# podmortem/log-parser

Hardware: AMD Instinct MI355X
Metric: log-lines/sec parsed+scored (whole node), 1k-pattern library (higher is better)
Workload: dtype fp64

## Files before the change

### csrc/bind.cpp

```cpp
#include <pybind11/numpy.h>
#include <pybind11/pybind11.h>
#include <pybind11/stl.h>

#include <atomic>
#include <chrono>
#include <condition_variable>
#include <cstring>
#include <deque>
#include <memory>
#include <mutex>
#include <thread>

#include "io/docs.h"
#include "io/json_in.h"
#include "io/loadgen.h"
#include "io/http_server.h"
#include "io/json_emit.h"
#include "kernels/lp_api.h"
#include "kernels/lp_host.h"
#include "regex/jregex.h"
#include "runtime/proc_shared.h"
#include "runtime/request.h"

namespace py = pybind11;
// ... 884 lines not shown
    bool intact = true;
    for (size_t i = k; i < out.size(); ++i) intact = intact && out[i] == '\xAB';
    return py::make_tuple(py::bytes(out.data(), k), intact);
  });

  m.def("line_index_tiles", &line_index_tiles);
  m.def("line_index_dev", [](uint64_t text, int64_t n, uint64_t ws, int64_t ntiles_cap, uint64_t starts, uint64_t lens,
                             int64_t cap, uint64_t info, bool trim, uint64_t blk, int64_t nblk, uint64_t s, bool counted) {
    line_index_dev(P<const uint8_t>(text), n, LineIndexWs{P<int64_t>(ws), ntiles_cap, size_t(1) << 20}, P<int64_t>(starts),
                   P<int32_t>(lens), cap, P<int64_t>(info), trim, P<int32_t>(blk), nblk, s, counted); },
        py::arg("text"), py::arg("n"), py::arg("ws"), py::arg("ntiles_cap"), py::arg("starts"), py::arg("lens"),
        py::arg("cap"), py::arg("info"), py::arg("trim"), py::arg("blk"), py::arg("nblk"), py::arg("s"),
        py::arg("counted") = false);
  m.def("prefilter_dev", [](uint64_t text, int64_t n, py::tuple pf, uint64_t ls, int64_t nl, uint64_t cand, int64_t cap,
                            uint64_t count, int grid, uint64_t s, py::object nlp) {
    NlOut o;
    const bool fused = !nlp.is_none();
    if (fused) {
      py::tuple t = nlp.cast<py::tuple>();
      o.nlm = P<uint64_t>(t[0].cast<uint64_t>());
      o.cnt = P<int32_t>(t[1].cast<uint64_t>());
      o.crf = P<int32_t>(t[2].cast<uint64_t>());
      o.ntiles = t[3].cast<int64_t>();
    }
    prefilter_dev(P<const uint8_t>(text), n, pf_from(pf), P<const int64_t>(ls), nl, P<int64_t>(cand), cap,
                  P<unsigned long long>(count), grid, s, fused ? &o : nullptr); },
        py::arg("text"), py::arg("n"), py::arg("pf"), py::arg("ls"), py::arg("nl"), py::arg("cand"), py::arg("cap"),
        py::arg("count"), py::arg("grid"), py::arg("s"), py::arg("nlp") = py::none());
  m.def("line_index_pass1", [](uint64_t ws, int64_t ntiles_cap, int64_t n, uint64_t s) {
    const NlOut o = line_index_pass1_views(LineIndexWs{P<int64_t>(ws), ntiles_cap, size_t(1) << 20}, n, s);
    return py::make_tuple(reinterpret_cast<uint64_t>(o.nlm), reinterpret_cast<uint64_t>(o.cnt),
                          reinterpret_cast<uint64_t>(o.crf), o.ntiles);
  });
  m.def("pf_verify_dev", [](uint64_t gh, int64_t n, uint64_t text, int64_t nb, py::tuple pf, uint64_t ls, int64_t nl,
                            uint64_t blk, uint64_t cand, int64_t cap, uint64_t count, uint64_t s, uint64_t dn,
                            int max_grid) {
    pf_verify_dev(P<const int64_t>(gh), n, P<const uint8_t>(text), nb, pf_from(pf), P<const int64_t>(ls), nl,
                  P<const int32_t>(blk), P<int64_t>(cand), cap, P<unsigned long long>(count), s,
                  P<const unsigned long long>(dn), max_grid); }, py::arg("gh"), py::arg("n"), py::arg("text"),
        py::arg("nb"), py::arg("pf"), py::arg("ls"), py::arg("nl"), py::arg("blk"), py::arg("cand"), py::arg("cap"),
        py::arg("count"), py::arg("s"), py::arg("dn") = 0, py::arg("max_grid") = 8192);
  m.def("append_keys", [](uint64_t dst, int64_t cap, uint64_t count, uint64_t src, int64_t n, uint64_t s) {
    append_keys_dev(P<int64_t>(dst), cap, P<unsigned long long>(count), P<const int64_t>(src), n, s); });
  m.def("take_host", [](uint64_t cand, uint64_t n1d, int64_t cap1, uint64_t ver, uint64_t n2d, int64_t cap2,
                        uint64_t text, uint64_t ls, uint64_t ll, py::tuple dfa, py::object out, uint64_t s) {
    HostSideOut O;
    if (!out.is_none()) {
      py::tuple t = out.cast<py::tuple>();
      O.keys = P<int64_t>(t[0].cast<uint64_t>()); O.starts = P<int64_t>(t[1].cast<uint64_t>());
      O.lens = P<int64_t>(t[2].cast<uint64_t>()); O.cap = t[3].cast<int64_t>();
      O.cnt = P<unsigned long long>(t[4].cast<uint64_t>()); O.done_blocks = P<unsigned int>(t[5].cast<uint64_t>());
      O.host_cnt = P<int64_t>(t[6].cast<uint64_t>()); O.host_seq = P<int64_t>(t[7].cast<uint64_t>());
      O.seq = t[8].cast<int64_t>();
    }
    take_host_dev(P<int64_t>(cand), P<const unsigned long long>(n1d), cap1, P<int64_t>(ver),
                  P<const unsigned long long>(n2d), cap2, P<const uint8_t>(text), P<const int64_t>(ls),
                  P<const int32_t>(ll), dfa_from(dfa), O, s); });
  m.def("wait_host", [](uint64_t ver, int64_t cap2, uint64_t n2d, py::tuple in, uint64_t s, double timeout_s) {
    HostSideIn I;
    I.keys = P<const int64_t>(in[0].cast<uint64_t>()); I.host_cnt = P<const int64_t>(in[1].cast<uint64_t>());
    I.host_seq = P<const int64_t>(in[2].cast<uint64_t>()); I.cap = in[3].cast<int64_t>(); I.seq = in[4].cast<int64_t>();
    I.err = P<int64_t>(in[5].cast<uint64_t>());
    I.timeout_ticks = (long long)(timeout_s * 1e8);
    wait_host_dev(P<int64_t>(ver), cap2, P<unsigned long long>(n2d), I, s); }, py::arg("ver"), py::arg("cap2"),
    py::arg("n2d"), py::arg("in"), py::arg("stream"), py::arg("timeout_s") = 2.0);
  m.def("host_alloc_coherent", [](int64_t bytes) {
// ... 284 lines not shown
        py::arg("hist"), py::arg("stream"), py::arg("dev"));
  m.def("trace_tile", &trace_tile);
  m.def("trace_runs_tmp_bytes", &trace_runs_tmp_bytes, py::arg("L"));
  m.def("trace_class", [](uint64_t text, int64_t tbytes, uint64_t ls, uint64_t ll, int64_t L, uint64_t cls, uint64_t elem,
                          uint64_t s, bool dev) {
    if (dev) {
      trace_class_dev(P<const uint8_t>(text), tbytes, P<const int64_t>(ls), P<const int32_t>(ll), L, P<uint8_t>(cls),
                      P<uint64_t>(elem), s);
      return;
    }
    py::gil_scoped_release nogil;
    trace_class_host(P<const uint8_t>(text), tbytes, P<const int64_t>(ls), P<const int32_t>(ll), L, P<uint8_t>(cls),
                     P<uint64_t>(elem)); },
        py::arg("text"), py::arg("tbytes"), py::arg("ls"), py::arg("ll"), py::arg("L"), py::arg("cls"), py::arg("elem"),
        py::arg("stream"), py::arg("dev"));
  m.def("trace_runs", [](uint64_t cls, uint64_t elem, uint64_t evm, int64_t L, std::vector<int64_t> carry, bool last,
                         uint64_t out, int64_t cap, uint64_t cnt, uint64_t carry_out, uint64_t tmp, uint64_t s, bool dev) {
    if ((int)carry.size() != TR_CARRY_WORDS) throw std::runtime_error("trace_runs: the carry has 13 words");
    TraceRunArgs A;
    A.cls = P<const uint8_t>(cls); A.elem = P<const uint64_t>(elem); A.evm = P<const uint8_t>(evm); A.L = L;
    A.in = TrCarry{carry[0], (uint64_t)carry[1], (uint64_t)carry[2], carry[3], carry[4], carry[5], carry[6], carry[7],
                   carry[8], carry[9], carry[10], carry[11], carry[12]};
    A.last = last;
    A.out = P<int64_t>(out); A.cap = cap; A.cnt = P<unsigned long long>(cnt); A.carry_out = P<int64_t>(carry_out);
    if (dev) {
      trace_runs_dev(A, P<void>(tmp), s);
      return;
    }
    py::gil_scoped_release nogil;
    trace_runs_host(A); },
        py::arg("cls"), py::arg("elem"), py::arg("evm"), py::arg("L"), py::arg("carry"), py::arg("last"), py::arg("out"),
        py::arg("cap"), py::arg("cnt"), py::arg("carry_out"), py::arg("tmp"), py::arg("stream"), py::arg("dev"));
  m.def("scan_multi", [](uint64_t text, int64_t nbytes, uint64_t ls, uint64_t ll, int64_t nl, py::tuple pass,
                         uint64_t out, int64_t cap, uint64_t cnt, int grid, uint64_t s, bool dev) -> int64_t {
    const ScanPass S = scan_pass_from(pass);
    if (dev) {
      scan_multi_dev(P<const uint8_t>(text), nbytes, P<const int64_t>(ls), P<const int32_t>(ll), nl, S, P<int64_t>(out), cap,
                     P<unsigned long long>(cnt), grid, s);
      return 0;
    }
    py::gil_scoped_release nogil;
    return scan_multi_host(P<const uint8_t>(text), P<const int64_t>(ls), P<const int32_t>(ll), nl, S, P<int64_t>(out),
                           cap);
  });
  m.def("freq_evict", [](py::tuple ring, double horizon, uint64_t s, bool dev) {
    freq_evict(ring_from(ring), horizon, s, dev);
  });
  m.def("summarize", [](py::tuple in, int64_t n, int k, int nsev, uint64_t top, uint64_t pat_hist, uint64_t sev_hist,
                        uint64_t ws, uint64_t ws_bytes, uint64_t s, bool dev) -> uint64_t {
    const SummIn I{P<const double>(in[0].cast<uint64_t>()), P<const int32_t>(in[1].cast<uint64_t>()),
                   P<const int32_t>(in[2].cast<uint64_t>()), P<const int64_t>(in[3].cast<uint64_t>()),
                   P<const int64_t>(in[4].cast<uint64_t>()), P<const int32_t>(in[5].cast<uint64_t>()),
                   P<const double>(in[6].cast<uint64_t>()),
                   in.size() > 7 ? P<void>(in[7].cast<uint64_t>()) : nullptr,
                   in.size() > 8 ? P<const int64_t>(in[8].cast<uint64_t>()) : nullptr};
    if (dev)
      return summarize_dev(I, n, k, nsev, P<double>(top), P<unsigned long long>(pat_hist), P<unsigned long long>(sev_hist),
                           P<void>(ws), ws_bytes, s);
    summarize_host(I, n, k, P<double>(top), P<int64_t>(pat_hist), P<int64_t>(sev_hist));
    return 0;
  });
  m.def("rescore", [](uint64_t gl, uint64_t fac, int64_t n, int64_t Nn, py::tuple sp, uint64_t out, uint64_t s,
                      bool dev) {
    if (dev)
      rescore_dev(P<const int64_t>(gl), P<const double>(fac), n, Nn, sp_from(sp), P<double>(out), s);
    else
      rescore_host(P<const int64_t>(gl), P<const double>(fac), n, Nn, sp_from(sp), P<double>(out));
  });
  m.def("dp_pack", [](int64_t own_lines, uint64_t freq, int nk, uint64_t chain, int ns, uint64_t pack, uint64_t s,
                      bool dev, uint64_t cnt, std::vector<int64_t> caps) {
    if (cnt && caps.size() != 4) throw std::invalid_argument("dp_pack: 4 capacities");
    dp_pack(own_lines, P<const int64_t>(freq), nk, P<const int32_t>(chain), ns, P<int64_t>(pack), s, dev,
            P<const int64_t>(cnt), cnt ? caps.data() : nullptr); },
        py::arg("own_lines"), py::arg("freq"), py::arg("nk"), py::arg("chain"), py::arg("ns"), py::arg("pack"),
        py::arg("s"), py::arg("dev"), py::arg("cnt") = 0, py::arg("caps") = std::vector<int64_t>());
  m.def("dp_carry", [](py::tuple a, uint64_t s, bool dev) {
    auto u = [&](int i) { return a[i].cast<uint64_t>(); };
// ... 454 lines not shown
```

### csrc/kernels/line_index.hip

```cpp
#include <hip/hip_runtime.h>

#include <cstring>
#include <stdexcept>
#include <string>

#include "lp_api.h"

namespace lp {

constexpr int LI_BYTES_PER_THREAD = 64;
__device__ __forceinline__ uint32_t li_zero_bytes(uint32_t t) {
  const uint32_t y = (t & 0x7F7F7F7Fu) + 0x7F7F7F7Fu;
  return ~(y | t | 0x7F7F7F7Fu);
}

constexpr int LI_THREADS = 256;
constexpr int LI_TILE = LI_THREADS * LI_BYTES_PER_THREAD;
constexpr int LI_STAGE = LI_THREADS * 8;

__device__ __forceinline__ int li_masks(const uint8_t* __restrict__ text, int64_t nbytes, int64_t base,
                                        uint32_t (&m)[16], uint32_t (&cr)[16]) {
  int c = 0;
  if (base < nbytes) {
    const uint4* p = reinterpret_cast<const uint4*>(text + base);
// ... 293 lines not shown
    for (int k = 0; k < LS_PER; ++k) {
      o[k] = run;
      run += cur[k];
    }
    if (i0 + LS_PER <= nt && ((uintptr_t)off & 15) == 0) {
      longlong2* o2 = reinterpret_cast<longlong2*>(off + i0);
#pragma unroll
      for (int k = 0; k < LS_PER / 2; ++k) o2[k] = make_longlong2(o[2 * k], o[2 * k + 1]);
    } else {
#pragma unroll
      for (int k = 0; k < LS_PER; ++k)
        if (i0 + k < nt) off[i0 + k] = o[k];
    }
    carry += tot;
#pragma unroll
    for (int k = 0; k < LS_PER; ++k) cur[k] = nxt[k];
  }
}

int64_t line_index_tiles(int64_t nbytes) { return (nbytes + LI_TILE - 1) / LI_TILE; }

NlOut line_index_pass1_views(const LineIndexWs& W, int64_t nbytes, uint64_t stream) {
  const int64_t nt = line_index_tiles(nbytes);
  if (nt <= 0 || nt > W.ntiles_cap) throw std::runtime_error("line_index: empty text or workspace too small");
  NlOut o;
  o.cnt = reinterpret_cast<int32_t*>(W.buf + 3 * W.ntiles_cap);
  o.crf = o.cnt + W.ntiles_cap;
  o.nlm = reinterpret_cast<uint64_t*>(W.buf + 4 * W.ntiles_cap);
  o.ntiles = nt;
  const hipError_t e = hipMemsetAsync(o.cnt, 0, (size_t)(W.ntiles_cap + nt) * sizeof(int32_t),
                                      reinterpret_cast<hipStream_t>(stream));
  if (e != hipSuccess) throw std::runtime_error(std::string("HIP error: ") + hipGetErrorString(e) + " in line_index");
  return o;
}

void line_index_dev(const uint8_t* text, int64_t nbytes, const LineIndexWs& W, int64_t* starts, int32_t* lens,
                    int64_t cap, int64_t* info, bool trim, int32_t* blk, int64_t nblk, uint64_t stream, bool counted) {
  const int64_t nt = line_index_tiles(nbytes);
  if (nt <= 0 || nt > W.ntiles_cap) throw std::runtime_error("line_index: empty text or workspace too small");
  hipStream_t st = reinterpret_cast<hipStream_t>(stream);
  int64_t* off = W.buf;
  int64_t* fix_g = W.buf + W.ntiles_cap;
  int64_t* fix_end = W.buf + 2 * W.ntiles_cap;
  int32_t* cnt = reinterpret_cast<int32_t*>(W.buf + 3 * W.ntiles_cap);
  int32_t* crf = cnt + W.ntiles_cap;
  uint64_t* nlm = reinterpret_cast<uint64_t*>(W.buf + 4 * W.ntiles_cap);
  if (!counted) hipLaunchKernelGGL(k_nl_count, dim3((unsigned)nt), dim3(LI_THREADS), 0, st, text, nbytes, cnt, nlm, crf);
  hipLaunchKernelGGL(k_tile_scan, dim3(1), dim3(LS_THREADS), 0, st, cnt, nt, off);
  hipLaunchKernelGGL(k_nl_lines, dim3((unsigned)((nt + LI_LINES_TPB - 1) / LI_LINES_TPB)), dim3(LI_THREADS), 0, st,
                     text, nbytes, (int64_t)nt, nlm, crf, off, starts, lens, cap,
                     fix_g, fix_end, blk, nblk);
  hipLaunchKernelGGL(k_line_fix, dim3((unsigned)((nt + 1 + 255) / 256)), dim3(256), 0, st, nt, nbytes, fix_g, fix_end,
                     off, cnt, starts, lens, cap, info, blk, nblk);
  if (trim) hipLaunchKernelGGL(k_line_trim, dim3(1), dim3(256), 0, st, lens, cap, info);
  const hipError_t e = hipGetLastError();
  if (e != hipSuccess) throw std::runtime_error(std::string("HIP error: ") + hipGetErrorString(e) + " in line_index");
}

}
```

### csrc/kernels/lp_api.h

```cpp
#pragma once
#include <stdint.h>

#include <vector>

#include "lp_core.h"

namespace lp {

void set_host_threads(int n);
void set_pf_verify_lanes(int n);
bool scan_defer_rare();
void set_scan_defer_rare(bool on);
void set_cand_verify_split(bool on);
bool summ_select();
void set_summ_select(bool on);
void set_small_profile(uint64_t dev_ptr);
struct NlOut {
  uint64_t* nlm = nullptr;
  int32_t* cnt = nullptr;
  int32_t* crf = nullptr;
  int64_t ntiles = 0;
};
void prefilter_dev(const uint8_t* text, int64_t nbytes, const PfTables& T, const int64_t* line_start, int64_t nlines,
                   int64_t* cand, int64_t cap, unsigned long long* count, int grid, uint64_t stream,
// ... 66 lines not shown
                const ScoreTables& T, const ScoreParams& S, double* out, double* factors);

}

namespace lp {
void nfa_mfma_dev(const uint64_t* groups, const int32_t* group_list, int ngroups, int ncls, const int32_t* lines,
                  int64_t nsel, const uint8_t* text, const int64_t* line_start, const int32_t* line_len,
                  uint8_t* feat, int64_t* hits, int64_t cap, unsigned long long* count, uint64_t stream);
int64_t nfa_host(const uint64_t* groups, const int32_t* group_list, int ngroups, const int32_t* lines, int64_t nsel,
                 const uint8_t* text, const int64_t* line_start, const int32_t* line_len, uint8_t* feat,
                 int64_t* hits, int64_t cap);
}

namespace lp {
struct ScanPass {
  const uint32_t* blob;
  int lds_words;
  int ngroups;
  int row_base[4];
  int stride[4];
  int thr[4];
  int init_row[4];
  uint32_t init_state[4];
  int ncol[4];
  int gt_off[4];
  int gm_off[4];
  int fin_off[4];
  int bm_off;
  int rid_off;
  int am_off;
};
void scan_multi_dev(const uint8_t* text, int64_t nbytes, const int64_t* line_start, const int32_t* line_len, int64_t nlines,
                    const ScanPass& S, int64_t* out, int64_t cap, unsigned long long* count, int grid,
                    uint64_t stream);
int64_t scan_multi_host(const uint8_t* text, const int64_t* line_start, const int32_t* line_len, int64_t nlines,
                        const ScanPass& S, int64_t* out, int64_t cap);
}

namespace lp {
struct FreqRing {
  double* t;
  int32_t* key;
  int32_t* cnt;
  int64_t cap;
  int64_t* ht;
  int64_t* tot;
  uint8_t* seen;
};
void freq_evict(const FreqRing& R, double horizon, uint64_t stream, bool dev);
struct RecordGate {
  const int64_t* cnt = nullptr;
  int64_t cap[4] = {0, 0, 0, 0};
  const int64_t* veto = nullptr;
};
void freq_record(const int64_t* counts, int K, double now, const FreqRing& R, uint64_t stream, bool dev,
                 const RecordGate& gate = RecordGate());
}

namespace lp {
struct LineIndexWs {
  int64_t* buf;
  int64_t ntiles_cap;
  size_t tmp_bytes;
};
int64_t line_index_tiles(int64_t nbytes);
void line_index_dev(const uint8_t* text, int64_t nbytes, const LineIndexWs& W, int64_t* starts, int32_t* lens,
                    int64_t cap, int64_t* info, bool trim, int32_t* blk, int64_t nblk, uint64_t stream,
                    bool counted = false);
NlOut line_index_pass1_views(const LineIndexWs& W, int64_t nbytes, uint64_t stream);
}

namespace lp {
struct DpCarryArgs {
  const int64_t* g;
  int world, rank, nk, ns;
  int64_t halo_left;
  const int64_t* tot;
  const int64_t* slot_e0;
  const int64_t* slot_k;
  int64_t* own_start; int64_t* g0; int64_t* n;
  int64_t* carry;
  uint8_t* seq_carry;
  int64_t* red_tail;
  int64_t* veto = nullptr;
  int64_t* zero = nullptr;
  int64_t nzero = 0;
  const uint8_t* seq_base = nullptr;
  int64_t line_base = 0;
  int64_t n_fixed = 0;
  uint8_t* seq_next = nullptr;
};
void dp_pack(int64_t own_lines, const int64_t* freq, int nk, const int32_t* chain, int ns, int64_t* pack,
             uint64_t stream, bool dev, const int64_t* cnt = nullptr, const int64_t* caps = nullptr);
void dp_carry(const DpCarryArgs& A, uint64_t stream, bool dev);
}

namespace lp {
struct SummIn {
  const double* score;
  const int32_t* pat;
  const int32_t* line32;
  const int64_t* line64;
// ... 279 lines not shown
```

### csrc/kernels/scan_multi.hip

```cpp
#include <hip/hip_runtime.h>

#include <map>
#include <mutex>
#include <stdexcept>
#include <string>
#include <utility>
#include <vector>

#include "lp_api.h"
#include "lp_core.h"
#include "lp_host.h"

namespace lp {

constexpr int SCAN_THREADS = 1024;
constexpr int SCAN_THREADS_SMALL = 256;
constexpr int SCAN_RUN = 4;
constexpr int SCAN_BM_COPIES = 32;
constexpr int SCAN_BM_REP_BYTES = 256 * SCAN_BM_COPIES * 4;

typedef __attribute__((address_space(3))) const uint16_t lds_u16_t;
typedef __attribute__((address_space(3))) const uint32_t lds_u32_t;
__device__ __forceinline__ uint32_t lds_ld16(uint32_t a) { return *(lds_u16_t*)(uintptr_t)a; }
__device__ __forceinline__ uint32_t lds_ld32(uint32_t a) { return *(lds_u32_t*)(uintptr_t)a; }
// ... 192 lines not shown
      } else {
        b = lds_ld32(c * 4);
      }
#pragma unroll
      for (int g = 0; g < G; ++g) {
        mx[g] = max(mx[g], xr[g]);
        xr[g] = lds_ld16(xr[g] + ((b >> (8 * g)) & 0xFFu));
      }
    }
    uint32_t hotm = 0;
#pragma unroll
    for (int g = 0; g < G; ++g) hotm |= (mx[g] >= (uint32_t)S.thr[g] ? 1u : 0u) << g;
    while (hotm) {
      const int g = __builtin_ctz(hotm);
      hotm &= hotm - 1;
      uint32_t xg = xs[0];
#pragma unroll
      for (int q = 1; q < G; ++q)
        if (g == q) xg = xs[q];
      if constexpr (DEFER) rare_push(rare, p0, p_lo, p_end, x0, x1, g, CRLF, xg);
      else scan_block_masks<CRLF>(S, w, hold, p0, p_lo, p_end, x0, x1, line_start, g, xg, emit);
    }
    cur = nxt;
    nxt = nx2;
  }
}

template <int G, int THREADS, bool DEFER>
__global__ __launch_bounds__(THREADS) void k_scan_multi(const uint8_t* __restrict__ text, int64_t nbytes,
                                                        const int64_t* __restrict__ line_start,
                                                        const int32_t* __restrict__ line_len, int64_t nlines,
                                                        ScanPass S, int64_t* __restrict__ out, int64_t cap,
                                                        unsigned long long* __restrict__ count, int run_len,
                                                        RareList rare) {
  extern __shared__ __attribute__((aligned(16))) uint32_t sm[];
  lds_fill<uint4>(reinterpret_cast<uint4*>(sm), reinterpret_cast<const uint4*>(S.blob), S.lds_words >> 2);
  constexpr bool REP = THREADS == SCAN_THREADS;
  uint32_t bm_rep = 0;
  if constexpr (REP) {
    uint32_t* rep = sm + S.lds_words;
    for (int i = threadIdx.x; i < 256 * SCAN_BM_COPIES; i += THREADS) rep[i] = S.blob[i / SCAN_BM_COPIES];
    bm_rep = (uint32_t)S.lds_words * 4 + (threadIdx.x & (SCAN_BM_COPIES - 1)) * 4;
  }
  __syncthreads();
  const GlobalEmit emit{out, cap, count};
  const bool at_zero = (uint32_t)(uintptr_t)(__attribute__((address_space(3))) uint32_t*)sm == 0u;
  const int64_t nruns = (nlines + run_len - 1) / run_len;
  const int64_t stride = (int64_t)gridDim.x * THREADS;
  struct Run {
    int64_t x0, x1, p_lo, p_end;
    bool fast, crlf;
  };
  auto prep = [&](int64_t run) {
    Run R;
    R.x0 = run * run_len;
    R.x1 = R.x0 + run_len < nlines ? R.x0 + run_len : nlines;
    R.fast = at_zero;
    R.crlf = false;
    if (run_len == SCAN_RUN && R.x0 + SCAN_RUN < nlines) {
      int64_t s5[SCAN_RUN + 1];
      int n4[SCAN_RUN];
#pragma unroll
      for (int i = 0; i <= SCAN_RUN; ++i) s5[i] = line_start[R.x0 + i];
#pragma unroll
      for (int i = 0; i < SCAN_RUN; ++i) n4[i] = line_len[R.x0 + i];
      bool term = false;
      int64_t sep = 1;
// ... 120 lines not shown
std::map<std::pair<int, uint64_t>, RareBuf> g_rare;

RareList rare_list(int64_t want, uint64_t stream) {
  int dev = 0;
  (void)hipGetDevice(&dev);
  std::lock_guard<std::mutex> lk(g_rare_mu);
  RareBuf& b = g_rare[{dev, stream}];
  if (b.need && *b.need > want) want = *b.need;
  if (!b.cnt) {
    if (hipMalloc(reinterpret_cast<void**>(&b.cnt), 16) != hipSuccess ||
        hipMemset(b.cnt, 0, 16) != hipSuccess ||
        hipHostMalloc(reinterpret_cast<void**>(&b.need), 8, hipHostMallocMapped | hipHostMallocCoherent) != hipSuccess)
      throw std::runtime_error("scan_multi: rare list allocation failed");
    *b.need = 0;
  }
  if (want > b.cap) {
    if (b.rec) (void)hipFree(b.rec);
    b.rec = nullptr;
    const int64_t cap = want + want / 4;
    if (hipMalloc(reinterpret_cast<void**>(&b.rec), (size_t)cap * RARE_WORDS * 8) != hipSuccess)
      throw std::runtime_error("scan_multi: rare list allocation failed");
    b.cap = cap;
    *b.need = 0;
  }
  int64_t* need_dev = nullptr;
  (void)hipHostGetDevicePointer(reinterpret_cast<void**>(&need_dev), b.need, 0);
  return RareList{b.rec, b.cap, b.cnt, reinterpret_cast<unsigned int*>(b.cnt + 1), need_dev};
}

}

void scan_multi_dev(const uint8_t* text, int64_t nbytes, const int64_t* line_start, const int32_t* line_len, int64_t nlines,
                    const ScanPass& S, int64_t* out, int64_t cap, unsigned long long* count, int grid,
                    uint64_t stream) {
  if (nlines <= 0 || S.ngroups <= 0) return;
  if (S.ngroups > 4 || (S.lds_words & 3) || S.lds_words * 4 + SCAN_BM_REP_BYTES > (160 << 10))
    throw std::runtime_error("scan_multi: bad pass descriptor");
  hipStream_t st = reinterpret_cast<hipStream_t>(stream);
  const bool small = nlines <= (int64_t)grid * SCAN_THREADS_SMALL;
  const size_t lds = (size_t)S.lds_words * 4 + (small ? 0 : SCAN_BM_REP_BYTES);
  const int64_t lanes = (int64_t)grid * SCAN_THREADS;
  const int run_len = small ? 1 : nlines < 2 * lanes ? 1 : nlines < 4 * lanes ? 2 : SCAN_RUN;
  const int threads = small ? SCAN_THREADS_SMALL : SCAN_THREADS;
  const int64_t runs = (nlines + run_len - 1) / run_len;
  const int64_t need = (runs + threads - 1) / threads;
  const int g = (int)std::max<int64_t>(1, std::min<int64_t>(small ? 4 * (int64_t)grid : grid, need));
  const bool defer = !small && scan_defer_rare();
  const RareList rare = defer ? rare_list(std::max<int64_t>(65536, runs), stream) : RareList{};
#define LP_SCAN(GV)                                                                                        \
  if (small)                                                                                               \
    hipLaunchKernelGGL((k_scan_multi<GV, SCAN_THREADS_SMALL, false>), dim3(g), dim3(SCAN_THREADS_SMALL), lds, st, \
                       text, nbytes, line_start, line_len, nlines, S, out, cap, count, run_len, rare);     \
  else if (defer)                                                                                          \
    hipLaunchKernelGGL((k_scan_multi<GV, SCAN_THREADS, true>), dim3(g), dim3(SCAN_THREADS), lds, st, text, \
                       nbytes, line_start, line_len, nlines, S, out, cap, count, run_len, rare);           \
  else                                                                                                     \
    hipLaunchKernelGGL((k_scan_multi<GV, SCAN_THREADS, false>), dim3(g), dim3(SCAN_THREADS), lds, st, text, \
                       nbytes, line_start, line_len, nlines, S, out, cap, count, run_len, rare)
  switch (S.ngroups) {
    case 1: LP_SCAN(1); break;
    case 2: LP_SCAN(2); break;
    case 3: LP_SCAN(3); break;
    default: LP_SCAN(4); break;
  }
#undef LP_SCAN
  hipError_t e = hipGetLastError();
  if (e != hipSuccess) throw std::runtime_error(std::string("HIP error: ") + hipGetErrorString(e) + " in scan_multi");
  if (defer) {
    hipLaunchKernelGGL(k_scan_rare, dim3(256), dim3(256), (size_t)S.lds_words * 4 + 32, st, text, line_start, S, out,
                       cap, count, rare);
    e = hipGetLastError();
    if (e != hipSuccess) throw std::runtime_error(std::string("HIP error: ") + hipGetErrorString(e) + " in scan_rare");
  }
}

int64_t scan_multi_host(const uint8_t* text, const int64_t* line_start, const int32_t* line_len, int64_t nlines,
                        const ScanPass& S, int64_t* out, int64_t cap) {
  const uint32_t* bm = S.blob + S.bm_off;
  std::vector<std::vector<int64_t>> part(std::max(1, host_threads()));
  host_parallel(nlines, 2048, [&](int th, int64_t a, int64_t b) {
    auto emit = [&](int64_t v) { part[th].push_back(v); };
    for (int64_t x = a; x < b; ++x) scan_line_exact(S, bm, text + line_start[x], line_len[x], x, emit);
  });
  int64_t c = 0;
  for (auto& v : part)
    for (int64_t k : v) {
      if (c < cap) out[c] = k;
      ++c;
    }
  return c;
}
// ... 3 lines not shown
```

### log_parser_amd/engine.py

```python
from __future__ import annotations

import logging
import os
import threading
import time
import uuid
import warnings
from dataclasses import dataclass, field
from datetime import datetime, timezone
from typing import Dict, List, Optional, Sequence, Tuple

import numpy as np
import torch

from .frequency import DeviceFrequencyState, FrequencyState
from .golden import SEVERITY_ORDER
from .models.compiled import CompiledLibrary
from .native import N, host_thread_budget
from .ops import kernels as K
from .utils import tracing as TR
from .utils.config import Config, ScoringParams

log = logging.getLogger("log_parser_amd.engine")

# ... 235 lines not shown
        try:
            return Stage(self.pinned, self.initial, self.initial // 16)
        except BaseException:
            with self._cv:
                self._out -= 1
                self._cv.notify()
            raise

    def give(self, st: Stage) -> None:
        with self._cv:
            self._out -= 1
            self._free.append(st)
            self._cv.notify()


class Engine:
    def __init__(self, library: CompiledLibrary, config: Optional[Config] = None,
                 device: Optional[torch.device] = None, freq: Optional[FrequencyState] = None):
        self.config = config or Config.load()
        self.lib = library
        self.params: ScoringParams = library.params
        self.device = device if device is not None else resolve_device(self.config["engine.device"])
        if freq is None:
            if self.device.type == "cuda" and bool(self.config.get("engine.frequency.device-resident", True)):
                freq = DeviceFrequencyState(library.freq_ids, self.params.freq_window_hours, self.device)
            else:
                freq = FrequencyState(self.params.freq_window_hours)
        self.freq = freq
        self.cand_cap = int(self.config["engine.candidate-capacity"])
        self.trace = bool(self.config.get("engine.trace", False))
        self.profile = self.trace
        self.context_engine = str(self.config["engine.context-engine"])
        self.log_matches = bool(self.config["server.log-matches"])
        self.fault_every = int(self.config["engine.fault-inject-every"])
        self.fault_after_record = int(self.config.get("engine.fault-inject-after-record", 0))
        self._batches = 0
        self.tabs = library.device_tables(self.device)
        self.ws = K.Workspace(self.device)
        self.arena = K.MatchArena()
        self.upload = K.Uploader(self.device)
        self.sp_tuple = self.score_param_tuple(self.params)
        self._pinned: Optional[torch.Tensor] = None
        self._stage_pool = StagePool(pinned=self.device.type == "cuda", initial=K.padded_len(1 << 20))
        self._side = None
        self._pf_stream = None
        self._doc_segs = None
        self._host_side = None
        self._runner = None
        if self.device.type == "cuda":
            props = torch.cuda.get_device_properties(self.device)
            self.n_cus = int(props.multi_processor_count)
            self.pf_grid = self.n_cus * 4
            if bool(self.config.get("engine.scan-stream", True)):
                self._side = (torch.cuda.Stream(self.device), torch.cuda.Event(), torch.cuda.Event())
            if bool(self.config.get("engine.prefilter-stream", True)):
                self._pf_stream = torch.cuda.Stream(self.device)
        else:
            self.n_cus = 1
            self.pf_grid = 1

    def stage_text(self, data: bytes) -> Tuple[torch.Tensor, int]:
        n = len(data)
        size = K.padded_len(n)
        src = _ro_view(data) if n else torch.empty(0, dtype=torch.uint8)
        if self.device.type == "cuda":
            if self._pinned is None or self._pinned.numel() < size:
                self._pinned = torch.empty(max(size, 1 << 20), dtype=torch.uint8, pin_memory=True)
            self._pinned[:n].copy_(src)
            self._pinned[n:size].zero_()
            dev = torch.empty(size, dtype=torch.uint8, device=self.device)
            dev.copy_(self._pinned[:size], non_blocking=True)
            return dev, n
        buf = torch.zeros(size, dtype=torch.uint8)
        buf[:n].copy_(src)
        return buf, n

    def _start(self, timings) -> float:
        if self.profile:
            TR.start(timings, self.device)
# ... 55 lines not shown
            ls_h = np.ascontiguousarray(ls_h, np.int64)
            ll_h = np.ascontiguousarray(ll_h, np.int32)
            lsp, llp, nl = ls_h.ctypes.data, ll_h.ctypes.data, ls_h.size
        else:
            lsp = llp = nl = 0
        loc, glob, lits = zip(*plan)
        keys = lib.host_bt.prepass(hb.ctypes.data, int(nbytes), lsp, llp, nl, trim, list(loc), list(glob),
                                   [list(x) for x in lits])
        if lib.host_bt.exhausted:
            log.warning("host backtracker: %d line matches exceeded the step budget (treated as no match)",
                        lib.host_bt.exhausted)
        return keys

    def scan_grid(self, sp: tuple) -> int:
        if self.device.type != "cuda":
            return 0
        per_cu = max(1, min(2, (160 << 10) // max(sp[1] * 4 + (32 << 10), 1)))
        return self.n_cus * per_cu

    def _ev_tables(self, segs: "Segments") -> tuple:
        return K.ev_tables(self.tabs, segs, len(self.lib.freq_ids), len(self.lib.patterns))

    def match_hits(self, text, nbytes, ls, ll, host_text=None, timings=None) -> torch.Tensor:
        cand, pre = self.match_candidates(text, nbytes, ls, ll, host_text, timings)
        segs = Segments.single(ls.numel(), text.device)
        return K.post_hits(cand, pre, ls.numel(), self.lib.n_regexes, text, ls, ll, self.tabs["dfa"],
                           self._ev_tables(segs), self.ws)[0]

    def prefilter_early(self, text, nbytes: int, nlp=None):
        if not text.is_cuda or self.profile:
            return None
        return K.EarlyPrefilter(text, nbytes, self.tabs, self.arena, self.pf_grid, nlp, stream=self._pf_stream)

    def split_with_prefilter(self, text, nbytes: int):
        box = []
        ls, ll = K.split_lines(text, nbytes, before_read=(lambda: box.append(self.prefilter_early(text, nbytes)))
                               if text.is_cuda else None, early_first=self._pf_stream is not None)
        return ls, ll, (box[0] if box else None)

    def fuses_line_index(self, text) -> bool:
        pf = self.lib.pf
        return (text.is_cuda and not self.profile and bool(self.config.get("engine.fused-line-index", False))
                and bool((pf["gmask"] & 28) or pf["teddy_lits"]))

    def can_defer(self, text) -> bool:
        import os
        return text.is_cuda and not self.profile and self.context_engine != "mfma"

    def prepare(self, text, nbytes, ls, ll, segs: Segments, host_text=None,
                timings: Optional[dict] = None, early=None, defer: bool = False,
                host_index: Optional[tuple] = None, split_trim: bool = True) -> "Prepared":
        timings = {} if timings is None else timings
        L = ls.numel()
        t = 0.0
        evt = self._ev_tables(segs)
        hs = None
        plan = None
        if self.lib.host_dev and text.is_cuda and host_text is not None:
            if self._host_side is None:
                from .ops.side_path import HostSide
                self._host_side = HostSide(self.lib, text.device,
                                           wait_s=float(self.config.get("engine.side-path-wait-s", 2.0)))
            self._host_side.check()
            if not self._host_side.take_fallback():
                hs = (self._host_side, np.asarray(host_text, dtype=np.uint8))
                plan = self.lib.host_plan_undev
        inj = self.host_hits(text, nbytes, host_text, *(host_index or (None, None)), trim=split_trim, plan=plan)
        if defer:
            hits, hit_line, hit_off, ev_cnt, ev_end, nh_cap, cnt, caps = K.match_and_hits(
                text, nbytes, ls, ll, self.tabs, self.lib.n_regexes, evt, self.arena, self.ws, self.pf_grid,
                self.scan_grid, side=self._side, early=early, defer=True, inject=inj, host_side=hs)
# ... 681 lines not shown
```

### log_parser_amd/ops/kernels.py

```python
from __future__ import annotations

from typing import Optional, Tuple

import torch

from ..native import N

TEXT_PAD = 64
NL_TILE = 16384


def _s(t: torch.Tensor) -> int:
    return torch.cuda.current_stream(t.device).cuda_stream if t.is_cuda else 0


def _p(t: Optional[torch.Tensor]) -> int:
    return 0 if t is None else t.data_ptr()


def padded_len(nbytes: int) -> int:
    return ((max(nbytes, 1) + NL_TILE - 1) // NL_TILE) * NL_TILE + TEXT_PAD


def newline_positions(text: torch.Tensor, nbytes: int) -> torch.Tensor:
# ... 8 lines not shown
    WORDS_PER_TILE = 4 + 256
    _all: dict = {}

    @classmethod
    def get(cls, text: torch.Tensor, ntiles: int) -> Tuple[int, int]:
        key = (text.device, _s(text))
        buf = cls._all.get(key)
        w = cls.WORDS_PER_TILE
        if buf is None or buf.numel() < w * ntiles + cls.SCAN_TMP // 8:
            cap = max(ntiles * 5 // 4, 1024)
            buf = cls._all[key] = torch.empty(w * cap + cls.SCAN_TMP // 8, dtype=torch.int64, device=text.device)
        return buf.data_ptr(), (buf.numel() - cls.SCAN_TMP // 8) // w


_LINES_PER_BYTE = [1.0 / 48]

import threading as _threading

_count_read = _threading.local()


def _count_read_slot(device: torch.device):
    slots = getattr(_count_read, "slots", None)
    if slots is None:
        slots = _count_read.slots = {}
    slot = slots.get(device.index)
    if slot is None:
        slot = slots[device.index] = (torch.empty(3, dtype=torch.int64, pin_memory=True), torch.cuda.Event())
    return slot
LINE_BLK_SHIFT = 12


def _line_index_dev(text: torch.Tensor, nbytes: int, trim: bool, before_read=None, fused=None,
                    early_first: bool = False):
    dev = text.device
    nt = N.line_index_tiles(nbytes)
    cap = int(nbytes * _LINES_PER_BYTE[0] * 1.25) + 1024
    blk = torch.empty((max(nbytes, 1) >> LINE_BLK_SHIFT) + 2, dtype=torch.int32, device=dev)
    counted = False
    while True:
        cap = min(cap, nbytes + 1)
        starts = torch.empty(cap, dtype=torch.int64, device=dev)
        lens = torch.empty(cap, dtype=torch.int32, device=dev)
        info = torch.empty(3, dtype=torch.int64, device=dev)
        wp, wcap = _LineIndexWs.get(text, nt)
        if fused is not None:
            fused(N.line_index_pass1(wp, wcap, nbytes, _s(text)))
            fused = None
            counted = True
        N.line_index_dev(text.data_ptr(), nbytes, wp, wcap, starts.data_ptr(), lens.data_ptr(), cap, info.data_ptr(),
                         trim, blk.data_ptr(), blk.numel(), _s(text), counted)
        if before_read is not None:
            if early_first:
                before_read()
            hinfo, done = _count_read_slot(dev)
            hinfo.copy_(info, non_blocking=True)
            done.record()
            if not early_first:
                before_read()
            before_read = None
            done.synchronize()
            n_nl, last, kept = hinfo.tolist()
        else:
            n_nl, last, kept = info.tolist()
        if n_nl + 1 <= cap:
            _LINES_PER_BYTE[0] = max(_LINES_PER_BYTE[0], (n_nl + 1) / max(nbytes, 1))
            return starts, lens, n_nl, last, kept, blk
        cap = n_nl + 1


def _with_blk(ls: torch.Tensor, blk: torch.Tensor, nbytes: int) -> torch.Tensor:
    ls._lp_blk = (blk, nbytes)
    return ls


def split_lines(text: torch.Tensor, nbytes: int, before_read=None, fused=None,
                early_first: bool = False) -> Tuple[torch.Tensor, torch.Tensor]:
    dev = text.device
    if text.is_cuda:
        if nbytes == 0:
            return torch.zeros(1, dtype=torch.int64, device=dev), torch.zeros(1, dtype=torch.int32, device=dev)
        starts, lens, _, _, L, blk = _line_index_dev(text, nbytes, trim=True, before_read=before_read, fused=fused,
                                                     early_first=early_first)
        return _with_blk(starts[:L], blk, nbytes), lens[:L]
    nl = newline_positions(text, nbytes)
    if nl.numel() == 0:
        return (torch.zeros(1, dtype=torch.int64, device=dev),
                torch.full((1,), nbytes, dtype=torch.int32, device=dev))
    zero = torch.zeros(1, dtype=torch.int64, device=dev)
    starts = torch.cat([zero, nl + 1])
    ends = torch.cat([nl, torch.full((1,), nbytes, dtype=torch.int64, device=dev)])
    prev = text[(nl - 1).clamp(min=0)]
    cr = (nl > starts[:-1]) & (prev == 13)
    ends[:-1] -= cr.to(torch.int64)
    lens = ends - starts
    nz = torch.nonzero(lens > 0)
    L = int(nz[-1].item()) + 1 if nz.numel() else 0
    return starts[:L].contiguous(), lens[:L].to(torch.int32).contiguous()


def split_chunk_lines(text: torch.Tensor, nbytes: int) -> Tuple[torch.Tensor, torch.Tensor]:
    dev = text.device
    if text.is_cuda and nbytes > 0:
        starts, lens, n_nl, last, _, blk = _line_index_dev(text, nbytes, trim=False)
        L = n_nl + 1 - (1 if n_nl and last == nbytes - 1 else 0)
        return _with_blk(starts[:L], blk, nbytes), lens[:L]
    nl = newline_positions(text.cpu(), nbytes).to(dev)
    zero = torch.zeros(1, dtype=torch.int64, device=dev)
    starts = torch.cat([zero, nl + 1])
    ends = torch.cat([nl, torch.full((1,), nbytes, dtype=torch.int64, device=dev)])
    if nl.numel():
        prev = text[(nl - 1).clamp(min=0)]
        cr = (nl > starts[:-1]) & (prev == 13)
        ends[:-1] -= cr.to(torch.int64)
    L = starts.numel()
    if nl.numel() and int(nl[-1].item()) == nbytes - 1:
# ... 217 lines not shown
        g, k, v, _, ne = counts
        return g > caps["gram"] or k > caps["cand"] or v > caps["ver"] or ne > caps["ev"]

    def learn_deferred(self, L: int, counts: list) -> None:
        g, k, v, nh, ne = counts
        self.last = {"lines": L, "gram_hits": g, "prefilter_candidates": k, "scan_hits": v, "hits": nh, "events": ne}
        self.learn(L, {"gram": g, "cand": k, "ver": v, "ev": ne}, overflow=False)

    def learn(self, L: int, counts: dict, overflow: bool) -> None:
        for k, c in counts.items():
            r = c / max(L, 1)
            self.rate[k] = max(r, self.rate[k] if overflow else self.rate[k] * 0.5, 1e-4)


def _pf_events(stream: "torch.cuda.Stream"):
    ev = getattr(_count_read, "pf_events", None)
    if ev is None:
        ev = _count_read.pf_events = {}
    e = ev.get(stream.cuda_stream)
    if e is None:
        e = ev[stream.cuda_stream] = (torch.cuda.Event(), torch.cuda.Event())
    return e


class EarlyPrefilter:

    def __init__(self, text, nbytes: int, tabs: dict, arena: "MatchArena", pf_grid: int, nlp=None,
                 stream: Optional["torch.cuda.Stream"] = None):
        L_est = int(nbytes * _LINES_PER_BYTE[0]) + 1
        self.cap = arena.caps(L_est)["gram"]
        self.gh = torch.empty(self.cap, dtype=torch.int64, device=text.device)
        self.cnt = torch.zeros(7, dtype=torch.int64, device=text.device)
        self.done = None
        st = _s(text)
        if stream is not None and nlp is None and text.is_cuda:
            fork, done = _pf_events(stream)
            fork.record(torch.cuda.current_stream(text.device))
            stream.wait_event(fork)
            st = stream.cuda_stream
        N.prefilter_dev(text.data_ptr(), nbytes, tabs["pf"], 0, 0, self.gh.data_ptr(), self.cap, self.cnt.data_ptr(),
                        pf_grid, st, nlp)
        if st != _s(text):
            self.done = done
            self.done.record(stream)
            for t in (self.gh, self.cnt, text):
                t.record_stream(stream)


def match_and_hits(text, nbytes: int, line_start, line_len, tabs: dict, R: int, evt: tuple, arena: MatchArena,
                   ws: Optional[Workspace], pf_grid: int, scan_grid, timings=None, tick=None, side=None,
                   early: Optional[EarlyPrefilter] = None, defer: bool = False,
                   inject: Optional[torch.Tensor] = None, host_side=None):
    dev = text.device
    L = line_start.numel()
    st = _s(text)
    lbits, rbits = N.bits_for(max(L, 1)), N.bits_for(max(R, 1))
    scans = bool(tabs["scan_passes"]) or bool(tabs["scan_regs"].numel()) or \
        any(g.numel() for g in tabs["nfa_scan_lists"].values())
    ninj = 0 if inject is None else inject.numel()
    for attempt in range(8):
        cap = arena.caps(L)
        cap["ver"] += ninj
        early_done = None
        if early is not None:
            cap["gram"] = early.cap
            gh, cnt = early.gh, early.cnt
            early_done = early.done
        else:
            gh = torch.empty(cap["gram"], dtype=torch.int64, device=dev)
            cnt = torch.zeros(7, dtype=torch.int64, device=dev)
        cand = torch.empty(cap["cand"], dtype=torch.int64, device=dev)
        ver = torch.empty(cap["ver"], dtype=torch.int64, device=dev)
        c0 = cnt.data_ptr()
        sst = st
        if side is not None and scans and tick is None:
            side[1].record()
            side[0].wait_event(side[1])
            sst = side[0].cuda_stream
        blk = line_block_index(line_start, nbytes)
        for sp in tabs["scan_passes"]:
            N.scan_multi(text.data_ptr(), nbytes, line_start.data_ptr(), line_len.data_ptr(), L, sp, ver.data_ptr(),
                         cap["ver"], c0 + 16, scan_grid(sp), sst, True)
        if tabs["scan_regs"].numel():
            N.scan_dev(text.data_ptr(), line_start.data_ptr(), line_len.data_ptr(), L, tabs["scan_regs"].data_ptr(),
                       tabs["scan_regs"].numel(), tabs["dfa"], ver.data_ptr(), cap["ver"], c0 + 16, sst)
        for ncls, glist in tabs["nfa_scan_lists"].items():
            if glist.numel():
                N.nfa(tabs["nfa_tables"].data_ptr(), glist.data_ptr(), glist.numel(), ncls, 0, L, text.data_ptr(),
                      line_start.data_ptr(), line_len.data_ptr(), 0, ver.data_ptr(), cap["ver"], c0 + 16, sst, True)
        if host_side is not None:
            host_side[0].begin(host_side[1])
            host_side[0].export_scan(ver, c0 + 16, cap["ver"], text, line_start, line_len, tabs["dfa"], sst)
        if sst != st:
            side[2].record(side[0])
        elif tick:
            tick("scan")
        if early is None:
            N.prefilter_dev(text.data_ptr(), nbytes, tabs["pf"], line_start.data_ptr(), L, gh.data_ptr(), cap["gram"],
                            c0, pf_grid, st)
        early = None
        if early_done is not None:
            torch.cuda.current_stream(dev).wait_event(early_done)
        N.pf_verify_dev(gh.data_ptr(), cap["gram"], text.data_ptr(), nbytes, tabs["pf"], line_start.data_ptr(), L,
                        blk.data_ptr(), cand.data_ptr(), cap["cand"], c0 + 8, st, c0,
                        max(16, min(8192, nbytes >> 13)))
        if tick:
            tick("prefilter")
        if host_side is not None:
            host_side[0].export_candidates(cand, c0 + 8, cap["cand"], text, line_start, line_len, tabs["dfa"], st)
        if sst != st:
            torch.cuda.current_stream(dev).wait_event(side[2])
        if host_side is not None:
            host_side[0].wait(ver, c0 + 16, cap["ver"], st)
        elif tabs.get("host_dev"):
            N.take_host(cand.data_ptr(), c0 + 8, cap["cand"], ver.data_ptr(), c0 + 16, cap["ver"], text.data_ptr(),
                        line_start.data_ptr(), line_len.data_ptr(), tabs["dfa"], None, st)
        if ninj:
            N.append_keys(ver.data_ptr(), cap["ver"], c0 + 16, inject.data_ptr(), ninj, st)
        n = cap["cand"] + cap["ver"]
        hits = torch.empty(n, dtype=torch.int64, device=dev)
        hit_line = torch.empty(n, dtype=torch.int32, device=dev)
        hit_off = torch.empty(R + 1, dtype=torch.int64, device=dev)
        ev_cnt = torch.empty(n, dtype=torch.int64, device=dev)
        ev_end = torch.empty(n, dtype=torch.int64, device=dev)

        def call(wp, wn):
            return N.post_hits(cand.data_ptr(), n, cap["cand"], lbits, rbits, R, text.data_ptr(),
# ... 753 lines not shown
```

### log_parser_amd/utils/config.py

```python
from __future__ import annotations

import os
import re
from dataclasses import dataclass, field
from typing import Any, Dict, Mapping, Optional

REFERENCE_KEYS: Dict[str, tuple] = {
    "pattern.directory": ("/shared/patterns", str),
    "scoring.proximity.decay-constant": (10.0, float),
    "scoring.proximity.max-window": (100, int),
    "scoring.chronological.early-bonus-threshold": (0.2, float),
    "scoring.chronological.max-early-bonus": (2.5, float),
    "scoring.chronological.penalty-threshold": (0.5, float),
    "scoring.context.max-context-factor": (2.5, float),
    "scoring.frequency.threshold": (10.0, float),
    "scoring.frequency.max-penalty": (0.8, float),
    "scoring.frequency.time-window-hours": (1, int),
}

ENGINE_KEYS: Dict[str, tuple] = {
    "engine.device": ("auto", str),
    "engine.serve-devices": ("", str),
    "engine.serve.peer-window": (False, bool),
    "engine.chunk-bytes": (0, int),
    "engine.stream.threshold-bytes": (256 << 20, int),
    "engine.candidate-capacity": (1 << 22, int),
    "engine.dfa-max-states": (2048, int),
    "engine.nfa-engine": ("bpg", str),
    "engine.context-engine": ("dfa", str),
    "engine.scan-stream": (False, bool),
    "engine.prefilter-stream": (True, bool),
    "engine.fused-line-index": (False, bool),
    "engine.native-runner": (True, bool),
    "engine.runner-device-counts": (True, bool),
    "engine.side-path-wait-s": (2.0, float),
    "engine.fallback-cpu": (True, bool),
    "engine.trace": (False, bool),
    "engine.fault-inject-every": (0, int),
    "engine.fault-inject-after-record": (0, int),
    "engine.batch.max-requests": (2048, int),
    "engine.batch.max-bytes": (256 << 20, int),
    "engine.batch.prewarm-bytes": (256 << 20, int),
    "engine.batch.max-wait-ms": (0.0, float),
    "engine.topk": (100, int),
    "engine.frequency.device-resident": (True, bool),
    "engine.frequency.snapshot-path": ("", str),
    "server.max-body-bytes": (1 << 30, int),
    "server.port": (8080, int),
    "server.host": ("0.0.0.0", str),
    "server.http": ("native", str),
    "server.io-threads": (0, int),
    "server.processes": (1, int),
    "server.max-restarts": (3, int),
    "server.numa-bind": (True, bool),
    "server.idle-timeout-s": (60.0, float),
    "server.l3-affinity": (True, bool),
    "server.prefetch-logs": (True, bool),
    "server.pinned-decode-buffers": (8, int),
    "server.io-decode-max-conns": (64, int),
    "server.io-spin-us": (0.0, float),
    "server.pump-spin-us": (1000.0, float),
    "server.tcp-quickack": (True, bool),
    "server.rcvbuf-bytes": (0, int),
    "server.trace-requests": (False, bool),
# ... 131 lines not shown
```

Before: 530.8 million.

## Launch prefilter after newline count and start scan passes before the line-count readback

Adds a standalone newline-count kernel so the early prefilter can be forked right after counting instead of after the full line index. It also adds an EarlyScan that launches the scan_multi passes immediately after the line index, before the host reads back the line count. The kernel clamps its line count from a device-side value. This is meant to overlap scanning with the host sync and the prefilter. In exchange it adds a speculative path that is discarded and rerun when the estimated line capacity is exceeded, plus more stream and event bookkeeping.

```diff
diff --git a/csrc/bind.cpp b/csrc/bind.cpp
--- a/csrc/bind.cpp
+++ b/csrc/bind.cpp
@@ -940,6 +940,9 @@
     return py::make_tuple(reinterpret_cast<uint64_t>(o.nlm), reinterpret_cast<uint64_t>(o.cnt),
                           reinterpret_cast<uint64_t>(o.crf), o.ntiles);
   });
+  m.def("line_index_count", [](uint64_t text, int64_t n, uint64_t ws, int64_t ntiles_cap, uint64_t s) {
+    line_index_count_dev(P<const uint8_t>(text), n, LineIndexWs{P<int64_t>(ws), ntiles_cap, size_t(1) << 20}, s);
+  });
   m.def("pf_verify_dev", [](uint64_t gh, int64_t n, uint64_t text, int64_t nb, py::tuple pf, uint64_t ls, int64_t nl,
                             uint64_t blk, uint64_t cand, int64_t cap, uint64_t count, uint64_t s, uint64_t dn,
                             int max_grid) {
@@ -1290,17 +1293,20 @@
         py::arg("cls"), py::arg("elem"), py::arg("evm"), py::arg("L"), py::arg("carry"), py::arg("last"), py::arg("out"),
         py::arg("cap"), py::arg("cnt"), py::arg("carry_out"), py::arg("tmp"), py::arg("stream"), py::arg("dev"));
   m.def("scan_multi", [](uint64_t text, int64_t nbytes, uint64_t ls, uint64_t ll, int64_t nl, py::tuple pass,
-                         uint64_t out, int64_t cap, uint64_t cnt, int grid, uint64_t s, bool dev) -> int64_t {
+                         uint64_t out, int64_t cap, uint64_t cnt, int grid, uint64_t s, bool dev,
+                         uint64_t dn) -> int64_t {
     const ScanPass S = scan_pass_from(pass);
     if (dev) {
       scan_multi_dev(P<const uint8_t>(text), nbytes, P<const int64_t>(ls), P<const int32_t>(ll), nl, S, P<int64_t>(out), cap,
-                     P<unsigned long long>(cnt), grid, s);
+                     P<unsigned long long>(cnt), grid, s, P<const int64_t>(dn));
       return 0;
     }
+    if (dn) throw std::runtime_error("scan_multi: a device line count needs the device path");
     py::gil_scoped_release nogil;
     return scan_multi_host(P<const uint8_t>(text), P<const int64_t>(ls), P<const int32_t>(ll), nl, S, P<int64_t>(out),
                            cap);
-  });
+  }, py::arg("text"), py::arg("nbytes"), py::arg("ls"), py::arg("ll"), py::arg("nl"), py::arg("pass"), py::arg("out"),
+        py::arg("cap"), py::arg("cnt"), py::arg("grid"), py::arg("s"), py::arg("dev"), py::arg("dn") = 0);
   m.def("freq_evict", [](py::tuple ring, double horizon, uint64_t s, bool dev) {
     freq_evict(ring_from(ring), horizon, s, dev);
   });
diff --git a/csrc/kernels/line_index.hip b/csrc/kernels/line_index.hip
--- a/csrc/kernels/line_index.hip
+++ b/csrc/kernels/line_index.hip
@@ -349,6 +349,18 @@
                                       reinterpret_cast<hipStream_t>(stream));
   if (e != hipSuccess) throw std::runtime_error(std::string("HIP error: ") + hipGetErrorString(e) + " in line_index");
   return o;
+}
+
+void line_index_count_dev(const uint8_t* text, int64_t nbytes, const LineIndexWs& W, uint64_t stream) {
+  const int64_t nt = line_index_tiles(nbytes);
+  if (nt <= 0 || nt > W.ntiles_cap) throw std::runtime_error("line_index: empty text or workspace too small");
+  int32_t* cnt = reinterpret_cast<int32_t*>(W.buf + 3 * W.ntiles_cap);
+  int32_t* crf = cnt + W.ntiles_cap;
+  uint64_t* nlm = reinterpret_cast<uint64_t*>(W.buf + 4 * W.ntiles_cap);
+  hipLaunchKernelGGL(k_nl_count, dim3((unsigned)nt), dim3(LI_THREADS), 0, reinterpret_cast<hipStream_t>(stream), text,
+                     nbytes, cnt, nlm, crf);
+  const hipError_t e = hipGetLastError();
+  if (e != hipSuccess) throw std::runtime_error(std::string("HIP error: ") + hipGetErrorString(e) + " in line_index");
 }
 
 void line_index_dev(const uint8_t* text, int64_t nbytes, const LineIndexWs& W, int64_t* starts, int32_t* lens,
diff --git a/csrc/kernels/lp_api.h b/csrc/kernels/lp_api.h
--- a/csrc/kernels/lp_api.h
+++ b/csrc/kernels/lp_api.h
@@ -122,7 +122,7 @@
 };
 void scan_multi_dev(const uint8_t* text, int64_t nbytes, const int64_t* line_start, const int32_t* line_len, int64_t nlines,
                     const ScanPass& S, int64_t* out, int64_t cap, unsigned long long* count, int grid,
-                    uint64_t stream);
+                    uint64_t stream, const int64_t* d_nlines = nullptr);
 int64_t scan_multi_host(const uint8_t* text, const int64_t* line_start, const int32_t* line_len, int64_t nlines,
                         const ScanPass& S, int64_t* out, int64_t cap);
 }
@@ -158,6 +158,7 @@
                     int64_t cap, int64_t* info, bool trim, int32_t* blk, int64_t nblk, uint64_t stream,
                     bool counted = false);
 NlOut line_index_pass1_views(const LineIndexWs& W, int64_t nbytes, uint64_t stream);
+void line_index_count_dev(const uint8_t* text, int64_t nbytes, const LineIndexWs& W, uint64_t stream);
 }
 
 namespace lp {
diff --git a/csrc/kernels/scan_multi.hip b/csrc/kernels/scan_multi.hip
--- a/csrc/kernels/scan_multi.hip
+++ b/csrc/kernels/scan_multi.hip
@@ -248,7 +248,11 @@
                                                         const int32_t* __restrict__ line_len, int64_t nlines,
                                                         ScanPass S, int64_t* __restrict__ out, int64_t cap,
                                                         unsigned long long* __restrict__ count, int run_len,
-                                                        RareList rare) {
+                                                        RareList rare, const int64_t* __restrict__ d_nlines) {
+  if (d_nlines) {
+    const int64_t dn = *d_nlines;
+    nlines = dn < nlines ? (dn > 0 ? dn : 0) : nlines;
+  }
   extern __shared__ __attribute__((aligned(16))) uint32_t sm[];
   lds_fill<uint4>(reinterpret_cast<uint4*>(sm), reinterpret_cast<const uint4*>(S.blob), S.lds_words >> 2);
   constexpr bool REP = THREADS == SCAN_THREADS;
@@ -435,7 +439,7 @@
 
 void scan_multi_dev(const uint8_t* text, int64_t nbytes, const int64_t* line_start, const int32_t* line_len, int64_t nlines,
                     const ScanPass& S, int64_t* out, int64_t cap, unsigned long long* count, int grid,
-                    uint64_t stream) {
+                    uint64_t stream, const int64_t* d_nlines) {
   if (nlines <= 0 || S.ngroups <= 0) return;
   if (S.ngroups > 4 || (S.lds_words & 3) || S.lds_words * 4 + SCAN_BM_REP_BYTES > (160 << 10))
     throw std::runtime_error("scan_multi: bad pass descriptor");
@@ -453,13 +457,13 @@
 #define LP_SCAN(GV)                                                                                        \
   if (small)                                                                                               \
     hipLaunchKernelGGL((k_scan_multi<GV, SCAN_THREADS_SMALL, false>), dim3(g), dim3(SCAN_THREADS_SMALL), lds, st, \
-                       text, nbytes, line_start, line_len, nlines, S, out, cap, count, run_len, rare);     \
+                       text, nbytes, line_start, line_len, nlines, S, out, cap, count, run_len, rare, d_nlines); \
   else if (defer)                                                                                          \
     hipLaunchKernelGGL((k_scan_multi<GV, SCAN_THREADS, true>), dim3(g), dim3(SCAN_THREADS), lds, st, text, \
-                       nbytes, line_start, line_len, nlines, S, out, cap, count, run_len, rare);           \
+                       nbytes, line_start, line_len, nlines, S, out, cap, count, run_len, rare, d_nlines); \
   else                                                                                                     \
     hipLaunchKernelGGL((k_scan_multi<GV, SCAN_THREADS, false>), dim3(g), dim3(SCAN_THREADS), lds, st, text, \
-                       nbytes, line_start, line_len, nlines, S, out, cap, count, run_len, rare)
+                       nbytes, line_start, line_len, nlines, S, out, cap, count, run_len, rare, d_nlines)
   switch (S.ngroups) {
     case 1: LP_SCAN(1); break;
     case 2: LP_SCAN(2); break;
diff --git a/log_parser_amd/engine.py b/log_parser_amd/engine.py
--- a/log_parser_amd/engine.py
+++ b/log_parser_amd/engine.py
@@ -291,6 +291,10 @@
         self.profile = self.trace
         self.context_engine = str(self.config["engine.context-engine"])
         self.log_matches = bool(self.config["server.log-matches"])
+        self.early_scan = bool(self.config.get("engine.early-scan", True))
+        self.prefilter_fork = str(self.config.get("engine.prefilter-fork", "count"))
+        if self.prefilter_fork not in ("index", "count", "start"):
+            raise ValueError("engine.prefilter-fork is one of index, count, start")
         self.fault_every = int(self.config["engine.fault-inject-every"])
         self.fault_after_record = int(self.config.get("engine.fault-inject-after-record", 0))
         self._batches = 0
@@ -304,6 +308,7 @@
         self._side = None
         self._pf_stream = None
         self._doc_segs = None
+        self.last_early_scan = None
         self._host_side = None
         self._runner = None
         if self.device.type == "cuda":
@@ -425,11 +430,38 @@
             return None
         return K.EarlyPrefilter(text, nbytes, self.tabs, self.arena, self.pf_grid, nlp, stream=self._pf_stream)
 
+    def early_scan_applies(self, text) -> bool:
+        return (text.is_cuda and not self.profile and self.early_scan and bool(self.tabs["scan_passes"])
+                and not self.lib.host_dev)
+
     def split_with_prefilter(self, text, nbytes: int):
-        box = []
-        ls, ll = K.split_lines(text, nbytes, before_read=(lambda: box.append(self.prefilter_early(text, nbytes)))
-                               if text.is_cuda else None, early_first=self._pf_stream is not None)
-        return ls, ll, (box[0] if box else None)
+        if not text.is_cuda or nbytes == 0:
+            ls, ll = K.split_lines(text, nbytes)
+            return ls, ll, None
+        fork = self.prefilter_fork if self._pf_stream is not None else "index"
+        box, reran = [], []
+
+        def prefilter():
+            box.append(self.prefilter_early(text, nbytes))
+
+        def scan(attempt, starts, lens, info):
+            early = box[0] if box else None
+            if attempt:
+                reran.append(attempt)
+            elif early is not None and self.early_scan_applies(text):
+                early.scan = K.EarlyScan(text, nbytes, starts, lens, info, self.tabs, self.arena, self.scan_grid,
+                                         early.cnt, side=self._side)
+
+        if fork == "start":
+            prefilter()
+        ls, ll = K.split_lines(text, nbytes, before_read=prefilter if fork == "index" else None,
+                               early_first=self._pf_stream is not None,
+                               after_count=prefilter if fork == "count" else None, after_index=scan)
+        early = box[0] if box else None
+        if early is not None and early.scan is not None and not early.scan.complete(ls.numel(), bool(reran)):
+            early.scan.discard(text.device)
+        self.last_early_scan = early.scan if early is not None else None
+        return ls, ll, early
 
     def fuses_line_index(self, text) -> bool:
         pf = self.lib.pf
diff --git a/log_parser_amd/ops/kernels.py b/log_parser_amd/ops/kernels.py
--- a/log_parser_amd/ops/kernels.py
+++ b/log_parser_amd/ops/kernels.py
@@ -64,12 +64,13 @@
 
 
 def _line_index_dev(text: torch.Tensor, nbytes: int, trim: bool, before_read=None, fused=None,
-                    early_first: bool = False):
+                    early_first: bool = False, after_count=None, after_index=None):
     dev = text.device
     nt = N.line_index_tiles(nbytes)
     cap = int(nbytes * _LINES_PER_BYTE[0] * 1.25) + 1024
     blk = torch.empty((max(nbytes, 1) >> LINE_BLK_SHIFT) + 2, dtype=torch.int32, device=dev)
     counted = False
+    attempt = 0
     while True:
         cap = min(cap, nbytes + 1)
         starts = torch.empty(cap, dtype=torch.int64, device=dev)
@@ -80,25 +81,34 @@
             fused(N.line_index_pass1(wp, wcap, nbytes, _s(text)))
             fused = None
             counted = True
+        elif after_count is not None and not counted:
+            N.line_index_count(text.data_ptr(), nbytes, wp, wcap, _s(text))
+            after_count()
+            counted = True
         N.line_index_dev(text.data_ptr(), nbytes, wp, wcap, starts.data_ptr(), lens.data_ptr(), cap, info.data_ptr(),
                          trim, blk.data_ptr(), blk.numel(), _s(text), counted)
-        if before_read is not None:
-            if early_first:
+        if before_read is not None or (after_index is not None and attempt == 0):
+            if early_first and before_read is not None:
                 before_read()
             hinfo, done = _count_read_slot(dev)
             hinfo.copy_(info, non_blocking=True)
             done.record()
-            if not early_first:
+            if not early_first and before_read is not None:
                 before_read()
             before_read = None
+            if after_index is not None:
+                after_index(attempt, starts, lens, info)
             done.synchronize()
             n_nl, last, kept = hinfo.tolist()
         else:
+            if after_index is not None:
+                after_index(attempt, starts, lens, info)
             n_nl, last, kept = info.tolist()
         if n_nl + 1 <= cap:
             _LINES_PER_BYTE[0] = max(_LINES_PER_BYTE[0], (n_nl + 1) / max(nbytes, 1))
             return starts, lens, n_nl, last, kept, blk
         cap = n_nl + 1
+        attempt += 1
 
 
 def _with_blk(ls: torch.Tensor, blk: torch.Tensor, nbytes: int) -> torch.Tensor:
@@ -107,13 +117,14 @@
 
 
 def split_lines(text: torch.Tensor, nbytes: int, before_read=None, fused=None,
-                early_first: bool = False) -> Tuple[torch.Tensor, torch.Tensor]:
+                early_first: bool = False, after_count=None, after_index=None) -> Tuple[torch.Tensor, torch.Tensor]:
     dev = text.device
     if text.is_cuda:
         if nbytes == 0:
             return torch.zeros(1, dtype=torch.int64, device=dev), torch.zeros(1, dtype=torch.int32, device=dev)
         starts, lens, _, _, L, blk = _line_index_dev(text, nbytes, trim=True, before_read=before_read, fused=fused,
-                                                     early_first=early_first)
+                                                     early_first=early_first, after_count=after_count,
+                                                     after_index=after_index)
         return _with_blk(starts[:L], blk, nbytes), lens[:L]
     nl = newline_positions(text, nbytes)
     if nl.numel() == 0:
@@ -397,6 +408,7 @@
         self.gh = torch.empty(self.cap, dtype=torch.int64, device=text.device)
         self.cnt = torch.zeros(7, dtype=torch.int64, device=text.device)
         self.done = None
+        self.scan: Optional["EarlyScan"] = None
         st = _s(text)
         if stream is not None and nlp is None and text.is_cuda:
             fork, done = _pf_events(stream)
@@ -410,6 +422,43 @@
             self.done.record(stream)
             for t in (self.gh, self.cnt, text):
                 t.record_stream(stream)
+
+
+class EarlyScan:
+
+    def __init__(self, text, nbytes: int, starts, lens, info, tabs: dict, arena: "MatchArena", scan_grid,
+                 cnt: torch.Tensor, side=None):
+        L_est = int(nbytes * _LINES_PER_BYTE[0]) + 1
+        self.lines_cap = max(1, min(starts.numel(), L_est))
+        self.cap = arena.caps(L_est)["ver"]
+        self.ver = torch.empty(self.cap, dtype=torch.int64, device=text.device)
+        self.cnt = cnt
+        self.index = (starts, lens, info)
+        self.join = None
+        self.discarded = False
+        st = _s(text)
+        if side is not None:
+            side[1].record()
+            side[0].wait_event(side[1])
+            st = side[0].cuda_stream
+        for sp in tabs["scan_passes"]:
+            N.scan_multi(text.data_ptr(), nbytes, starts.data_ptr(), lens.data_ptr(), self.lines_cap, sp,
+                         self.ver.data_ptr(), self.cap, cnt.data_ptr() + 16, scan_grid(sp), st, True,
+                         info.data_ptr() + 16)
+        if side is not None:
+            self.join = side[2]
+            self.join.record(side[0])
+            for t in (self.ver, cnt, text, starts, lens, info):
+                t.record_stream(side[0])
+
+    def complete(self, L: int, reran: bool) -> bool:
+        return not reran and L <= self.lines_cap
+
+    def discard(self, device) -> None:
+        if self.join is not None:
+            torch.cuda.current_stream(device).wait_event(self.join)
+        self.cnt[2:3].zero_()
+        self.discarded = True
 
 
 def match_and_hits(text, nbytes: int, line_start, line_len, tabs: dict, R: int, evt: tuple, arena: MatchArena,
@@ -427,23 +476,35 @@
         cap = arena.caps(L)
         cap["ver"] += ninj
         early_done = None
+        es = None
         if early is not None:
             cap["gram"] = early.cap
             gh, cnt = early.gh, early.cnt
             early_done = early.done
+            es = early.scan
+            if es is not None and es.discarded:
+                es = None
         else:
             gh = torch.empty(cap["gram"], dtype=torch.int64, device=dev)
             cnt = torch.zeros(7, dtype=torch.int64, device=dev)
         cand = torch.empty(cap["cand"], dtype=torch.int64, device=dev)
-        ver = torch.empty(cap["ver"], dtype=torch.int64, device=dev)
+        if es is not None:
+            cap["ver"] = es.cap
+            ver = es.ver
+        else:
+            ver = torch.empty(cap["ver"], dtype=torch.int64, device=dev)
         c0 = cnt.data_ptr()
         sst = st
-        if side is not None and scans and tick is None:
+        later = bool(tabs["scan_regs"].numel()) or any(g.numel() for g in tabs["nfa_scan_lists"].values())
+        if es is not None and not later:
+            if es.join is not None:
+                sst = side[0].cuda_stream
+        elif side is not None and scans and tick is None:
             side[1].record()
             side[0].wait_event(side[1])
             sst = side[0].cuda_stream
         blk = line_block_index(line_start, nbytes)
-        for sp in tabs["scan_passes"]:
+        for sp in (tabs["scan_passes"] if es is None else ()):
             N.scan_multi(text.data_ptr(), nbytes, line_start.data_ptr(), line_len.data_ptr(), L, sp, ver.data_ptr(),
                          cap["ver"], c0 + 16, scan_grid(sp), sst, True)
         if tabs["scan_regs"].numel():
@@ -457,7 +518,8 @@
             host_side[0].begin(host_side[1])
             host_side[0].export_scan(ver, c0 + 16, cap["ver"], text, line_start, line_len, tabs["dfa"], sst)
         if sst != st:
-            side[2].record(side[0])
+            if es is None or later:
+                side[2].record(side[0])
         elif tick:
             tick("scan")
         if early is None:
diff --git a/log_parser_amd/utils/config.py b/log_parser_amd/utils/config.py
--- a/log_parser_amd/utils/config.py
+++ b/log_parser_amd/utils/config.py
@@ -30,6 +30,8 @@
     "engine.context-engine": ("dfa", str),
     "engine.scan-stream": (False, bool),
     "engine.prefilter-stream": (True, bool),
+    "engine.prefilter-fork": ("count", str),
+    "engine.early-scan": (True, bool),
     "engine.fused-line-index": (False, bool),
     "engine.native-runner": (True, bool),
     "engine.runner-device-counts": (True, bool),
```

Result: no change. 529.7 million (-0.2%).
